# shibatch/rectdetect

Hardware: AMD Instinct MI355X
Metric: 1920x1080 frames/sec (higher is better)
Workload: dtype u8/i32/f32 (bit-exact integer + IEEE f32 stencil path)

## Files before the change

### rectdetect_amd/csrc/rd_k_front.hip

```cpp
#include <stdlib.h>
#include "rd_device.h"
#include "rd_kernels.h"
#include "rectdetect_hip.h"

#define RD_LUT_ATTR __device__
#include "rd_luts.h"

namespace {

using namespace rd;
using namespace rdpix;

struct P3 { float *p[3]; };
struct P3c { const float *p[3]; };
struct SrcZ { const uint8_t *p[RD_ZB_MAX]; };

inline int cdiv(int a, int b) { return (a + b - 1) / b; }
inline dim3 grid2(int iw, int ih) { return dim3(cdiv(iw, 64), cdiv(ih, 4)); }
const dim3 block2(64, 4);
inline int grid1(int n) { int g = cdiv(n, 256); return g < 1 ? 1 : g; }

__device__ __forceinline__ int lerp_lut(const unsigned short *t, int c) { return t[c >> 8] * (256 - (c & 255)) + t[(c >> 8) + 1] * (c & 255); }

__device__ __forceinline__ uint32_t plab_of(const unsigned short *s_s2l, const unsigned short *s_cf, const unsigned short *s_cf2, int b, int g, int r) {
  const int ib = s_s2l[b], ig = s_s2l[g], ir = s_s2l[r];
  const int cx = (((ir * 6758 + ig * 5859 + ib * 2956 + (1 << 14)) >> 15) * 34476 + (1 << 10)) >> 11;
  const int cy = ((ir * 3484 + ig * 11717 + ib * 1182) + (1 << 10)) >> 11;
  const int cz = (((ir * 317 + ig * 1953 + ib * 15569 + (1 << 14)) >> 15) * 30097 + (1 << 10)) >> 11;
  const int cl = ((lerp_lut(s_cf2, cy) >> 12) + 1) >> 1;
  const int fx = lerp_lut(s_cf, cx), fy = lerp_lut(s_cf, cy), fz = lerp_lut(s_cf, cz);
  const int fxy = (fx - fy + (1 << 7)) >> 8, fyz = (fy - fz + (1 << 7)) >> 8;
  const int ca = (fxy * 8031 + (134744072 + (1 << 17))) >> 18;
  const int cb = (fyz * 3213 + (134744072 + (1 << 17))) >> 18;
  uint32_t v = clampu((uint32_t)cb, 0u, 1023u);
  v = (v << 10) | clampu((uint32_t)ca, 0u, 1023u);
  v = (v << 12) | clampu((uint32_t)cl, 0u, 4095u);
  return v;
}

__global__ __launch_bounds__(256) void k_bgr2plab(uint32_t *__restrict__ out, const uint8_t *__restrict__ bgr, int iw, int ih, int ws) {
  __shared__ unsigned short s_s2l[RD_LUT_S2L_N], s_cf[RD_LUT_CF_N], s_cf2[RD_LUT_CF_N];
  const int tid = rd_ty() * 64 + threadIdx.x;
  for (int i = tid; i < RD_LUT_S2L_N; i += 256) s_s2l[i] = rd_lut_s2l[i];
  for (int i = tid; i < RD_LUT_CF_N; i += 256) { s_cf[i] = rd_lut_cfunc[i]; s_cf2[i] = rd_lut_cfunc2[i]; }
  __syncthreads();
  const int x = blockIdx.x * 64 + threadIdx.x;
  if (x >= iw) return;
  for (int r = 0; r < 4; r++) {
    const int y = (blockIdx.y * 4 + rd_ty()) * 4 + r;
    if (y >= ih) break;
    const uint8_t *p = bgr + (size_t)y * ws + x * 3;
    const int ib = s_s2l[p[0]], ig = s_s2l[p[1]], ir = s_s2l[p[2]];
    const int cx = (((ir * 6758 + ig * 5859 + ib * 2956 + (1 << 14)) >> 15) * 34476 + (1 << 10)) >> 11;
    const int cy = ((ir * 3484 + ig * 11717 + ib * 1182) + (1 << 10)) >> 11;
    const int cz = (((ir * 317 + ig * 1953 + ib * 15569 + (1 << 14)) >> 15) * 30097 + (1 << 10)) >> 11;
    const int cl = ((lerp_lut(s_cf2, cy) >> 12) + 1) >> 1;
    const int fx = lerp_lut(s_cf, cx), fy = lerp_lut(s_cf, cy), fz = lerp_lut(s_cf, cz);
    const int fxy = (fx - fy + (1 << 7)) >> 8, fyz = (fy - fz + (1 << 7)) >> 8;
    const int ca = (fxy * 8031 + (134744072 + (1 << 17))) >> 18;
    const int cb = (fyz * 3213 + (134744072 + (1 << 17))) >> 18;
    uint32_t v = clampu((uint32_t)cb, 0u, 1023u);
    v = (v << 10) | clampu((uint32_t)ca, 0u, 1023u);
    v = (v << 12) | clampu((uint32_t)cl, 0u, 4095u);
    out[y * iw + x] = v;
  }
}

__global__ __launch_bounds__(256) void k_bgr2plab_t(uint32_t *__restrict__ out, P3 dst, SrcZ srcz, int iw, int ih, int ws, size_t zs) {
  const uint8_t *__restrict__ bgr = srcz.p[blockIdx.z];
  RD_ZSHIFT(zs, out, dst.p[0], dst.p[1], dst.p[2]);
  __shared__ unsigned short s_s2l[RD_LUT_S2L_N], s_cf[RD_LUT_CF_N], s_cf2[RD_LUT_CF_N];
  __shared__ unsigned short tile[3][64][66];
  const int tid = rd_ty() * 64 + threadIdx.x;
  const int x0 = blockIdx.x * 64, y0 = blockIdx.y * 64;
  const int x = x0 + threadIdx.x;
  uint8_t pb[16], pg[16], pr[16];
#pragma unroll
  for (int k = 0; k < 16; k++) {
    const int y = y0 + rd_ty() + 4 * k;
    const uint8_t *p = bgr + ((x < iw && y < ih) ? (size_t)y * ws + x * 3 : 0);
    pb[k] = p[0]; pg[k] = p[1]; pr[k] = p[2];
  }
  for (int i = tid; i < RD_LUT_S2L_N; i += 256) s_s2l[i] = rd_lut_s2l[i];
  for (int i = tid; i < RD_LUT_CF_N; i += 256) { s_cf[i] = rd_lut_cfunc[i]; s_cf2[i] = rd_lut_cfunc2[i]; }
  __syncthreads();
#pragma unroll
  for (int k = 0; k < 16; k++) {
    const int r = rd_ty() + 4 * k;
    const int y = y0 + r;
    if (x >= iw || y >= ih) continue;
    const int ib = s_s2l[pb[k]], ig = s_s2l[pg[k]], ir = s_s2l[pr[k]];
    const int cx = (((ir * 6758 + ig * 5859 + ib * 2956 + (1 << 14)) >> 15) * 34476 + (1 << 10)) >> 11;
    const int cy = ((ir * 3484 + ig * 11717 + ib * 1182) + (1 << 10)) >> 11;
    const int cz = (((ir * 317 + ig * 1953 + ib * 15569 + (1 << 14)) >> 15) * 30097 + (1 << 10)) >> 11;
    const int cl = ((lerp_lut(s_cf2, cy) >> 12) + 1) >> 1;
    const int fx = lerp_lut(s_cf, cx), fy = lerp_lut(s_cf, cy), fz = lerp_lut(s_cf, cz);
    const int fxy = (fx - fy + (1 << 7)) >> 8, fyz = (fy - fz + (1 << 7)) >> 8;
    const int ca = (fxy * 8031 + (134744072 + (1 << 17))) >> 18;
    const int cb = (fyz * 3213 + (134744072 + (1 << 17))) >> 18;
    uint32_t v = clampu((uint32_t)cb, 0u, 1023u);
    v = (v << 10) | clampu((uint32_t)ca, 0u, 1023u);
    v = (v << 12) | clampu((uint32_t)cl, 0u, 4095u);
    out[y * iw + x] = v;
    tile[0][r][threadIdx.x] = (unsigned short)(v & 4095u); tile[1][r][threadIdx.x] = (unsigned short)((v >> 12) & 1023u); tile[2][r][threadIdx.x] = (unsigned short)((v >> 22) & 1023u);
  }
  __syncthreads();
  for (int r = rd_ty(); r < 64; r += 4) {
    const int ox = y0 + threadIdx.x, oy = x0 + r;
    if (ox < ih && oy < iw)
      for (int k = 0; k < 3; k++) ((unsigned short *)dst.p[k])[(size_t)oy * ih + ox] = tile[k][threadIdx.x][r];
  }
}

struct PixZ { const uint8_t *p[3][RD_ZB_MAX]; int pitch[3]; int wide; };

__device__ __forceinline__ uint32_t ld_bytes(const uint8_t *p, int n) {
  uint32_t w = 0;
#pragma unroll
  for (int i = 0; i < 4; i++) if (i < n) w |= (uint32_t)p[i] << (8 * i);
  return w;
}
template <int FMT> __device__ __forceinline__ void pix_load4(uint32_t (&w)[4], const uint8_t *p0, const uint8_t *p1, const uint8_t *p2, const int (&pitch)[3], int x, int y, int m, bool wide) {
  if (rdpix::bpp(FMT) == 3) {
    const uint8_t *q = p0 + (size_t)y * pitch[0] + 3 * x;
    if (wide && m == 4) { const uint32_t *q4 = (const uint32_t *)q; w[0] = q4[0]; w[1] = q4[1]; w[2] = q4[2]; }
    else for (int k = 0; k < 3; k++) w[k] = ld_bytes(q + 4 * k, 3 * m - 4 * k);
  } else if (rdpix::bpp(FMT) == 4) {
    const uint8_t *q = p0 + (size_t)y * pitch[0] + 4 * x;
    if (wide && m == 4) { const uint4 v = *(const uint4 *)q; w[0] = v.x; w[1] = v.y; w[2] = v.z; w[3] = v.w; }
    else for (int k = 0; k < 4; k++) w[k] = ld_bytes(q + 4 * k, k < m ? 4 : 0);
  } else {
    const uint8_t *q = p0 + (size_t)y * pitch[0] + x;
    const int c = (m + 1) >> 1;
    if (FMT == RD_PIX_NV12) {
      const uint8_t *uv = p1 + (size_t)(y >> 1) * pitch[1] + x;
      if (wide && m == 4) { w[0] = *(const uint32_t *)q; w[1] = *(const uint32_t *)uv; }
      else { w[0] = ld_bytes(q, m); w[1] = ld_bytes(uv, 2 * c); }
    } else {
      const uint8_t *u = p1 + (size_t)(y >> 1) * pitch[1] + (x >> 1), *v = p2 + (size_t)(y >> 1) * pitch[2] + (x >> 1);
      if (wide && m == 4) { w[0] = *(const uint32_t *)q; w[1] = (uint32_t)*(const unsigned short *)u | ((uint32_t)*(const unsigned short *)v << 16); }
      else { w[0] = ld_bytes(q, m); w[1] = ld_bytes(u, c) | (ld_bytes(v, c) << 16); }
    }
  }
}

template <int FMT> __device__ __forceinline__ void pix_bgr(const uint32_t (&w)[4], int j, int &b, int &g, int &r) {
  const auto byte = [&](int i) { return (int)((w[i >> 2] >> (8 * (i & 3))) & 255u); };
  if (!is_yuv(FMT)) {
    const int i = rdpix::bpp(FMT) * j, c[3] = { byte(i), byte(i + 1), byte(i + 2) };
    b = c[rb_swapped(FMT) ? 2 : 0]; g = c[1]; r = c[rb_swapped(FMT) ? 0 : 2];
  } else if (FMT == RD_PIX_NV12) yuv_bgr(byte(j), byte(4 + 2 * (j >> 1)), byte(5 + 2 * (j >> 1)), b, g, r);
  else yuv_bgr(byte(j), byte(4 + (j >> 1)), byte(6 + (j >> 1)), b, g, r);
}

template <int FMT>
__global__ __launch_bounds__(256) void k_pix2plab_t(uint32_t *__restrict__ out, P3 dst, PixZ src, int iw, int ih, size_t zs) {
  const int z = blockIdx.z;
  const uint8_t *__restrict__ p0 = src.p[0][z], *__restrict__ p1 = src.p[1][z], *__restrict__ p2 = src.p[2][z];
  RD_ZSHIFT(zs, out, dst.p[0], dst.p[1], dst.p[2]);
  __shared__ unsigned short s_s2l[RD_LUT_S2L_N], s_cf[RD_LUT_CF_N], s_cf2[RD_LUT_CF_N];
  __shared__ unsigned short tile[3][64][66];
  const int tid = rd_ty() * 64 + threadIdx.x;
  const int x0 = blockIdx.x * 64, y0 = blockIdx.y * 64;
  const int cx = (tid & 15) * 4, r0 = tid >> 4;
  const int x = x0 + cx, m = min(iw - x, 4);
  uint32_t w[4][4] = {};
#pragma unroll
  for (int k = 0; k < 4; k++) {
    const int y = y0 + r0 + 16 * k;
    if (m > 0 && y < ih) pix_load4<FMT>(w[k], p0, p1, p2, src.pitch, x, y, m, src.wide != 0);
  }
  for (int i = tid; i < RD_LUT_S2L_N; i += 256) s_s2l[i] = rd_lut_s2l[i];
  for (int i = tid; i < RD_LUT_CF_N; i += 256) { s_cf[i] = rd_lut_cfunc[i]; s_cf2[i] = rd_lut_cfunc2[i]; }
  __syncthreads();
#pragma unroll
  for (int k = 0; k < 4; k++) {
    const int r = r0 + 16 * k, y = y0 + r;
    if (m <= 0 || y >= ih) continue;
    uint32_t v[4];
#pragma unroll
    for (int j = 0; j < 4; j++) {
      int b, g, rr;
      pix_bgr<FMT>(w[k], j, b, g, rr);
      v[j] = plab_of(s_s2l, s_cf, s_cf2, b, g, rr);
      tile[0][r][cx + j] = (unsigned short)(v[j] & 4095u); tile[1][r][cx + j] = (unsigned short)((v[j] >> 12) & 1023u); tile[2][r][cx + j] = (unsigned short)((v[j] >> 22) & 1023u);
    }
    uint32_t *o = out + (size_t)y * iw + x;
    if (m == 4 && (iw & 3) == 0) *(uint4 *)o = make_uint4(v[0], v[1], v[2], v[3]);
    else for (int j = 0; j < m; j++) o[j] = v[j];
  }
  __syncthreads();
  for (int r = rd_ty(); r < 64; r += 4) {
    const int ox = y0 + threadIdx.x, oy = x0 + r;
    if (ox < ih && oy < iw)
      for (int k = 0; k < 3; k++) ((unsigned short *)dst.p[k])[(size_t)oy * ih + ox] = tile[k][threadIdx.x][r];
  }
}

template <int FMT> struct HalfW { static constexpr int row = 2 * rdpix::bpp(FMT), n = is_yuv(FMT) ? 6 : 2 * row; };

template <int FMT> __device__ __forceinline__ void pix_load_half(uint32_t (&w)[HalfW<FMT>::n], const uint8_t *p0, const uint8_t *p1, const uint8_t *p2, const int (&pitch)[3], int x, int y, int m, bool wide) {
  constexpr int RW = HalfW<FMT>::row;
  const bool full = wide && m == 4;
  if (!is_yuv(FMT)) {
    constexpr int bpp = rdpix::bpp(FMT);
    const uint8_t *q = p0 + (size_t)(2 * y) * pitch[0] + (size_t)(2 * x) * bpp;
#pragma unroll
    for (int r = 0; r < 2; r++, q += pitch[0]) {
      if (full) {
        if (bpp == 4) { const uint4 a = ((const uint4 *)q)[0], b = ((const uint4 *)q)[1]; w[RW * r] = a.x; w[RW * r + 1] = a.y; w[RW * r + 2] = a.z; w[RW * r + 3] = a.w; w[RW * r + 4] = b.x; w[RW * r + 5] = b.y; w[RW * r + 6] = b.z; w[RW * r + 7] = b.w; }
        else { const uint2 a = ((const uint2 *)q)[0], b = ((const uint2 *)q)[1], c = ((const uint2 *)q)[2]; w[RW * r] = a.x; w[RW * r + 1] = a.y; w[RW * r + 2] = b.x; w[RW * r + 3] = b.y; w[RW * r + 4] = c.x; w[RW * r + 5] = c.y; }
      } else {
#pragma unroll
        for (int k = 0; k < RW; k++) w[RW * r + k] = ld_bytes(q + 4 * k, 2 * m * bpp - 4 * k);
      }
    }
  } else {
    const uint8_t *q = p0 + (size_t)(2 * y) * pitch[0] + 2 * x;
#pragma unroll
    for (int r = 0; r < 2; r++, q += pitch[0]) {
      if (full) { const uint2 a = *(const uint2 *)q; w[2 * r] = a.x; w[2 * r + 1] = a.y; }
      else { w[2 * r] = ld_bytes(q, 2 * m); w[2 * r + 1] = ld_bytes(q + 4, 2 * m - 4); }
    }
    if (FMT == RD_PIX_NV12) {
      const uint8_t *uv = p1 + (size_t)y * pitch[1] + 2 * x;
      if (full) { const uint2 a = *(const uint2 *)uv; w[4] = a.x; w[5] = a.y; }
      else { w[4] = ld_bytes(uv, 2 * m); w[5] = ld_bytes(uv + 4, 2 * m - 4); }
    } else {
      const uint8_t *u = p1 + (size_t)y * pitch[1] + x, *v = p2 + (size_t)y * pitch[2] + x;
      if (full) { w[4] = *(const uint32_t *)u; w[5] = *(const uint32_t *)v; }
      else { w[4] = ld_bytes(u, m); w[5] = ld_bytes(v, m); }
    }
  }
}

template <int FMT> __device__ __forceinline__ void pix_bgr_half(const uint32_t (&w)[HalfW<FMT>::n], int j, int &b, int &g, int &r) {
  constexpr int RW = HalfW<FMT>::row;
  const auto byte = [&](int i) { return (int)((w[i >> 2] >> (8 * (i & 3))) & 255u); };
  b = g = r = 2;
#pragma unroll
  for (int t = 0; t < 4; t++) {
    const int sx = 2 * j + (t & 1), sr = t >> 1;
    int pb, pg, pr;
    if (!is_yuv(FMT)) {
      const int i = 4 * RW * sr + rdpix::bpp(FMT) * sx, c[3] = { byte(i), byte(i + 1), byte(i + 2) };
      pb = c[rb_swapped(FMT) ? 2 : 0]; pg = c[1]; pr = c[rb_swapped(FMT) ? 0 : 2];
    } else if (FMT == RD_PIX_NV12) yuv_bgr(byte(8 * sr + sx), byte(16 + 2 * j), byte(17 + 2 * j), pb, pg, pr);
    else yuv_bgr(byte(8 * sr + sx), byte(16 + j), byte(20 + j), pb, pg, pr);
    b += pb; g += pg; r += pr;
  }
  b >>= 2; g >>= 2; r >>= 2;
}

template <int FMT>
__global__ __launch_bounds__(256) void k_pix2plab_half_t(uint32_t *__restrict__ out, P3 dst, PixZ src, int iw, int ih, size_t zs) {
  const int z = blockIdx.z;
  const uint8_t *__restrict__ p0 = src.p[0][z], *__restrict__ p1 = src.p[1][z], *__restrict__ p2 = src.p[2][z];
  RD_ZSHIFT(zs, out, dst.p[0], dst.p[1], dst.p[2]);
  __shared__ unsigned short s_s2l[RD_LUT_S2L_N], s_cf[RD_LUT_CF_N], s_cf2[RD_LUT_CF_N];
  __shared__ unsigned short tile[3][64][66];
  const int tid = rd_ty() * 64 + threadIdx.x;
  const int x0 = blockIdx.x * 64, y0 = blockIdx.y * 64;
  const int cx = (tid & 15) * 4, r0 = tid >> 4;
  const int x = x0 + cx, m = min(iw - x, 4);
  uint32_t w[4][HalfW<FMT>::n] = {};
#pragma unroll
  for (int k = 0; k < 4; k++) {
    const int y = y0 + r0 + 16 * k;
    if (m > 0 && y < ih) pix_load_half<FMT>(w[k], p0, p1, p2, src.pitch, x, y, m, src.wide != 0);
  }
  for (int i = tid; i < RD_LUT_S2L_N; i += 256) s_s2l[i] = rd_lut_s2l[i];
  for (int i = tid; i < RD_LUT_CF_N; i += 256) { s_cf[i] = rd_lut_cfunc[i]; s_cf2[i] = rd_lut_cfunc2[i]; }
  __syncthreads();
#pragma unroll
  for (int k = 0; k < 4; k++) {
    const int r = r0 + 16 * k, y = y0 + r;
    if (m <= 0 || y >= ih) continue;
    uint32_t v[4];
#pragma unroll
    for (int j = 0; j < 4; j++) {
      int b, g, rr;
      pix_bgr_half<FMT>(w[k], j, b, g, rr);
      v[j] = plab_of(s_s2l, s_cf, s_cf2, b, g, rr);
      tile[0][r][cx + j] = (unsigned short)(v[j] & 4095u); tile[1][r][cx + j] = (unsigned short)((v[j] >> 12) & 1023u); tile[2][r][cx + j] = (unsigned short)((v[j] >> 22) & 1023u);
    }
    uint32_t *o = out + (size_t)y * iw + x;
    if (m == 4 && (iw & 3) == 0) *(uint4 *)o = make_uint4(v[0], v[1], v[2], v[3]);
    else for (int j = 0; j < m; j++) o[j] = v[j];
  }
  __syncthreads();
  for (int r = rd_ty(); r < 64; r += 4) {
    const int ox = y0 + threadIdx.x, oy = x0 + r;
    if (ox < ih && oy < iw)
      for (int k = 0; k < 3; k++) ((unsigned short *)dst.p[k])[(size_t)oy * ih + ox] = tile[k][threadIdx.x][r];
  }
}

template <typename LD, typename ST> __device__ __forceinline__ void ew4(int n, LD ld, ST st) {
  const int stride = gridDim.x * blockDim.x;
  int i = blockIdx.x * blockDim.x + threadIdx.x;
  for (; i + 3 * stride < n; i += 4 * stride) {
    const auto v0 = ld(i), v1 = ld(i + stride), v2 = ld(i + 2 * stride), v3 = ld(i + 3 * stride);
    st(i, v0); st(i + stride, v1); st(i + 2 * stride, v2); st(i + 3 * stride, v3);
  }
  for (; i < n; i += stride) st(i, ld(i));
}

__global__ void k_unpack_plab(float *__restrict__ L, float *__restrict__ a, float *__restrict__ b, const uint32_t *__restrict__ in, int n) {
  for (int i = blockIdx.x * blockDim.x + threadIdx.x; i < n; i += gridDim.x * blockDim.x) {
    float l, aa, bb;
    unpack_lab(in[i], l, aa, bb);
    L[i] = l; a[i] = aa; b[i] = bb;
  }
}

__global__ void k_pack_plab(uint32_t *__restrict__ out, const float *__restrict__ L, const float *__restrict__ a, const float *__restrict__ b, int n) {
  ew4(n, [=](int i) { return make_float3(L[i], a[i], b[i]); }, [=](int i, float3 v) { out[i] = pack_lab(v.x, v.y, v.z); });
}

template <int MODE>
__global__ __launch_bounds__(256) void k_transpose(P3 dst, P3c src, P3c fwd, P3c bwd, const uint32_t *__restrict__ plab, int np, int W, int H, const int *only_if) {
  if (only_if && *only_if == 0) return;
  __shared__ float tile[3][64][65];
  const int x0 = blockIdx.x * 64, y0 = blockIdx.y * 64;
  for (int r = rd_ty(); r < 64; r += 4) {
    const int x = x0 + threadIdx.x, y = y0 + r;
    if (x < W && y < H) {
      const size_t i = (size_t)y * W + x;
// ... 141 lines not shown
          if (xin && yy >= s0 && yy < s0 + 7) IIR_OUT(tl + (size_t)(3 * 7 + yy - s0) * W) = d;
          IIR_SHIFT(cur[j]);
        }
#pragma unroll
        for (int j = 0; j < IIR_CH; j++) cur[j] = nxt[j];
      }
    }
  }
  if (TOUT) {
    __syncthreads();
    const int rows = s1 - s0;
    for (int col = anti; col < 64; col += 2) {
      const int xx = blockIdx.x * 64 + col;
      if (xx >= W) break;
      float *__restrict__ o = dk + (size_t)xx * H + s0;
      for (int r = lane; r < rows; r += 64) at32(o, (unsigned)r) = fwt[r * IF_PITCH + col];
    }
  }
}

__device__ __forceinline__ unsigned iir_off(unsigned o) { asm("" : "+v"(o)); return o; }
template <typename T> __device__ __forceinline__ __attribute__((address_space(1))) T *iir_uni(T *p) {
  __attribute__((address_space(1))) T *g = (__attribute__((address_space(1))) T *)p;
  asm("" : "+s"(g));
  return g;
}
#ifndef IIR_PCH
#define IIR_PCH 16
#endif
#ifndef IF_TB
#define IF_TB 32
#endif
#define IF_TP (64 + 64 / IF_TB)
#ifdef IF_WPE
#define IF_WPE_ATTR __attribute__((amdgpu_waves_per_eu(IF_WPE)))
#else
#define IF_WPE_ATTR
#endif
template <int TOUT, int IF_ROWS, int SRC16>
__global__ __launch_bounds__(128) IF_WPE_ATTR void k_iir_fused(P3 dst, P3c src, float *__restrict__ tails, int W, int H, int nchunks, int *bad, int np, size_t zs) {
  constexpr int HALF = IF_ROWS / 2, CH = IIR_PCH, CPI = 64 / IF_TB;
  static_assert(CH >= 8 && IF_WU % CH == 0 && HALF % CH == 0 && HALF % IF_TB == 0 && 64 % IF_TB == 0, "whole chunks and whole batches, half a block per phase");
  __shared__ float swp[2 * 14 * 64];
  __shared__ float stg[TOUT ? 2 * IF_TB * IF_TP : 1];
  const int lane = threadIdx.x & 63, anti = __builtin_amdgcn_readfirstlane((int)(threadIdx.x >> 6));
  const int fz = __builtin_amdgcn_readfirstlane((int)(blockIdx.y / np)), k = blockIdx.y - fz * np, c = blockIdx.z;
  float *dk = k == 0 ? dst.p[0] : (k == 1 ? dst.p[1] : dst.p[2]);
  const float *sk = k == 0 ? src.p[0] : (k == 1 ? src.p[1] : src.p[2]);
  { const size_t rd_zoff_ = (size_t)fz * zs; RD_ZS1(dk); RD_ZS1(sk); RD_ZS1(tails); RD_ZS1(bad); }
  if (blockIdx.x == 0 && k == 0 && blockIdx.z == 0 && threadIdx.x == 0) *bad = 0;
  const int x = blockIdx.x * 64 + lane;
  const bool xin = x < W;
  typedef typename iir_src<SRC16>::T TS;
  const TS *__restrict__ in = (const TS *)sk;
  const unsigned xs = (unsigned)(xin ? x : W - 1) * (unsigned)sizeof(TS), x4 = (unsigned)(xin ? x : W - 1) * 4u;
#undef IIR_ROW
#undef IIR_OUT
#define IIR_ROW(ptr) (*(const TS *)((const char *)(ptr) + xo_))
#define IIR_OUT(ptr) (*(float *)((char *)(ptr) + iir_off(x4)))
  const float sc = k == 0 ? 1.0f / 4096 : 1.0f / 1024, hf = k == 0 ? 0.5f / 4096 : 0.5f / 1024;
  const int s0 = c * IF_ROWS, s1 = s0 + IF_ROWS, mid = s0 + HALF;
  float *__restrict__ tl = tails + ((size_t)(k * nchunks + c) * 4 * 7) * W;
  const long rs = anti ? -(long)W : (long)W;
  float cur[CH], nxt[CH], park[HALF];
#define IIR_PSTEPS(...)                                                                                                  \
      _Pragma("unroll") for (int j = 0; j < CH; j++) {                                                                   \
        IIR_STEP(cur[j]);                                                                                                \
        __VA_ARGS__;                                                                                                     \
        IIR_SHIFT(cur[j]);                                                                                               \
      }                                                                                                                  \
      _Pragma("unroll") for (int j = 0; j < CH; j++) cur[j] = nxt[j];
#define IIR_PCHUNK(MORE, NEXT, NSTEP, ...)                                                                               \
    {                                                                                                                    \
      if (MORE) { const TS *n_ = (NEXT); const unsigned xo_ = iir_off(xs); _Pragma("unroll") for (int j = 0; j < CH; j++) { nxt[j] = IIR_LD(IIR_ROW(iir_uni(n_))); n_ += (NSTEP); } } \
      IIR_PSTEPS(__VA_ARGS__)                                                                                            \
    }
#define IIR_PARK(dst, v) asm("v_mov_b32 %0, %1" : "=v"(dst) : "v"(v))
  IIR_STATE;
  const TS *p = in + (size_t)(anti ? s1 - 1 : s0) * W;
  const TS *const pb = in + (size_t)(anti ? mid : mid - 1) * W;
  float *const tw = tl + (size_t)(anti ? 2 * 7 + 6 : 0) * W;
#define IIR_WTAIL if (j >= CH - 7 && xin) IIR_OUT(iir_uni(tw + (long)(j - (CH - 7)) * rs)) = d
  if (anti ? s1 + IF_WU <= H : s0 - IF_WU >= 0) {
    const TS *w = p - IF_WU * rs;
    { const unsigned xo_ = iir_off(xs);
#pragma unroll
      for (int j = 0; j < CH; j++) cur[j] = IIR_LD(IIR_ROW(iir_uni(w + (long)j * rs))); }
    for (int q = 0; q < IF_WU / CH - 1; q++) { IIR_PCHUNK(1, w + CH * rs, rs, (void)0); w += CH * rs; }
    IIR_PCHUNK(1, p, rs, IIR_WTAIL);
  } else {
    const int dy = anti ? -1 : 1, y0 = anti ? s1 - 1 + IF_WU : s0 - IF_WU;
    const unsigned xo_ = iir_off(xs);
    auto eld = [&](int yy) -> float {
      const int yc = clampi(yy, -IIR_WARM, H + IIR_WARM);
      const float v = IIR_LD(IIR_ROW(iir_uni(in + (size_t)mirror1(yc, H) * W)));
      return yy == yc ? v : 0.0f;
    };
#define IIR_PCHUNK_E(YN, ...) { _Pragma("unroll") for (int j = 0; j < CH; j++) nxt[j] = eld((YN) + j * dy); IIR_PSTEPS(__VA_ARGS__) }
#pragma unroll
    for (int j = 0; j < CH; j++) cur[j] = eld(y0 + j * dy);
    for (int q = 0; q < IF_WU / CH - 1; q++) IIR_PCHUNK_E(y0 + (q + 1) * CH * dy, (void)0)
    IIR_PCHUNK(1, p, rs, IIR_WTAIL);
  }
#undef IIR_WTAIL
#pragma unroll
  for (int q = 0; q < HALF / CH; q++) {
    const bool last = q == HALF / CH - 1;
    IIR_PCHUNK(1, last ? pb : p + CH * rs, last ? -rs : rs, IIR_PARK(park[q * CH + j], d)); p += CH * rs;
  }
  {
    float *mine = swp + anti * (14 * 64) + lane, *theirs = swp + (anti ^ 1) * (14 * 64) + lane;
#define IIR_SWAP(n, q) mine[(2 * n) * 64] = q.x; mine[(2 * n + 1) * 64] = q.y;
    IIR_SWAP(0, q1) IIR_SWAP(1, q2) IIR_SWAP(2, q3) IIR_SWAP(3, q4) IIR_SWAP(4, q5) IIR_SWAP(5, q6) IIR_SWAP(6, q7)
#undef IIR_SWAP
    __syncthreads();
#define IIR_SWAP(n, q) q.x = theirs[(2 * n) * 64]; q.y = theirs[(2 * n + 1) * 64];
    IIR_SWAP(0, q1) IIR_SWAP(1, q2) IIR_SWAP(2, q3) IIR_SWAP(3, q4) IIR_SWAP(4, q5) IIR_SWAP(5, q6) IIR_SWAP(6, q7)
#undef IIR_SWAP
  }
  p = pb;
  float *const tt = tl + (size_t)(anti ? 1 * 7 : 3 * 7 + 6) * W;
  float *o = dk + (size_t)(anti ? mid : mid - 1) * W;
  float *const st = stg + (TOUT ? anti * (IF_TB * IF_TP) : 0);
  const int br = lane % IF_TB, bc = lane / IF_TB;
  const float *const sl = st + (anti ? br : IF_TB - 1 - br) * IF_TP + bc;
  const unsigned bo = ((unsigned)bc * (unsigned)H + (unsigned)br) * 4u;
#pragma unroll
  for (int q = 0; q < HALF / CH; q++) {
    const bool last = q == HALF / CH - 1;
    IIR_PCHUNK(!last, p - CH * rs, -rs, {
      const int i = q * CH + j;
      const float r = (park[HALF - 1 - i] + d) - cur[j] * IIR_C0;
      if (TOUT) st[(i % IF_TB) * IF_TP + lane] = r; else if (xin) IIR_OUT(iir_uni(o - (long)j * rs)) = r;
      if (i >= HALF - 7 && xin) IIR_OUT(iir_uni(tt - (long)(i - (HALF - 7)) * rs)) = d;
      if (TOUT && i % IF_TB == IF_TB - 1) {
        __builtin_amdgcn_fence(__ATOMIC_RELEASE, "wavefront"); __builtin_amdgcn_wave_barrier(); __builtin_amdgcn_fence(__ATOMIC_ACQUIRE, "wavefront");
        const int lowest = anti ? mid + (i / IF_TB) * IF_TB : mid - (i / IF_TB + 1) * IF_TB;
        float *const ob = dk + (size_t)(blockIdx.x * 64) * H + lowest;
        _Pragma("unroll") for (int n = 0; n < IF_TB; n++)
          if ((int)blockIdx.x * 64 + n * CPI + bc < W) *(float *)((char *)iir_uni(ob + (size_t)(n * CPI) * H) + bo) = sl[n * CPI];
        __builtin_amdgcn_fence(__ATOMIC_RELEASE, "wavefront"); __builtin_amdgcn_wave_barrier(); __builtin_amdgcn_fence(__ATOMIC_ACQUIRE, "wavefront");
      }
    });
    p -= CH * rs; if (!TOUT) o -= CH * rs;
  }
#undef IIR_PCHUNK
#undef IIR_PCHUNK_E
#undef IIR_PSTEPS
#undef IIR_PARK
}

#undef IIR_LD
#undef IIR_ROW
#undef IIR_OUT

#define IC_CH 4
template <int TOUT, int SRC16, int EAGER>
__global__ __launch_bounds__(64 * IC_CH) void k_iir_check_fix(P3 dst, P3c src, P3 fwd, const float *__restrict__ tails, int *bad, int W, int H, int nchunks, int IF_ROWS, int force, int np, size_t zs) {
  const int x = blockIdx.x * 64 + threadIdx.x;
  const int k = blockIdx.y % np, c = blockIdx.z * IC_CH + rd_ty();
  if (c >= nchunks) return;
  float *dk = k == 0 ? dst.p[0] : (k == 1 ? dst.p[1] : dst.p[2]), *fk = k == 0 ? fwd.p[0] : (k == 1 ? fwd.p[1] : fwd.p[2]);
  const float *sk = k == 0 ? src.p[0] : (k == 1 ? src.p[1] : src.p[2]);
  { const size_t rd_zoff_ = (size_t)(blockIdx.y / np) * zs; RD_ZS1(dk); RD_ZS1(sk); RD_ZS1(fk); RD_ZS1(tails); RD_ZS1(bad); }
  if (x >= W) return;
  const int s0 = c * IF_ROWS, s1 = (c == nchunks - 1) ? H : s0 + IF_ROWS;
  const float *me = tails + ((size_t)(k * nchunks + c) * 4 * 7) * W + x;
  bool differ = force != 0 && c == 0;
  const bool chk_f = c > 0 && s0 - IF_WU > -IIR_WARM;
  const bool chk_b = c < nchunks - 1 && s1 - 1 + IF_WU < H + IIR_WARM;
  const float *pv = tails + ((size_t)(k * nchunks + (chk_f ? c - 1 : c)) * 4 * 7) * W + x;
  const float *nx = tails + ((size_t)(k * nchunks + (chk_b ? c + 1 : c)) * 4 * 7) * W + x;
  if (EAGER) {
    unsigned a[14], b[14];
#pragma unroll
    for (int j = 0; j < 7; j++) {
      a[j] = __float_as_uint(me[(size_t)(0 * 7 + j) * W]); b[j] = __float_as_uint(pv[(size_t)(1 * 7 + j) * W]);
      a[7 + j] = __float_as_uint(me[(size_t)(2 * 7 + j) * W]); b[7 + j] = __float_as_uint(nx[(size_t)(3 * 7 + j) * W]);
    }
    unsigned df = 0, db = 0;
#pragma unroll
    for (int j = 0; j < 7; j++) { df |= a[j] ^ b[j]; db |= a[7 + j] ^ b[7 + j]; }
    differ = differ || (chk_f && df != 0) || (chk_b && db != 0);
  } else {
    if (chk_f) {
#pragma unroll
      for (int j = 0; j < 7; j++) differ = differ || (__float_as_uint(me[(size_t)(0 * 7 + j) * W]) != __float_as_uint(pv[(size_t)(1 * 7 + j) * W]));
    }
    if (chk_b) {
#pragma unroll
      for (int j = 0; j < 7; j++) differ = differ || (__float_as_uint(me[(size_t)(2 * 7 + j) * W]) != __float_as_uint(nx[(size_t)(3 * 7 + j) * W]));
    }
  }
  if (!differ) return;
  atomicOr(bad, 1);
  typedef typename iir_src<SRC16>::T TS;
  const TS *__restrict__ in = (const TS *)sk + x;
  const float sc = k == 0 ? 1.0f / 4096 : 1.0f / 1024, hf = k == 0 ? 0.5f / 4096 : 0.5f / 1024;
  float *fw = fk + x;
  {
    IIR_STATE;
    for (int yy = -IIR_WARM; yy < H; yy++) {
      const float i0 = iir_field<SRC16>(in[(size_t)mirror1(yy, H) * W], sc, hf);
// ... 380 lines not shown
  }
  return z;
}
void pix2plab_transposed(hipStream_t s, int fmt, uint32_t *out, float *const dst[3], const uint8_t *const (*planes)[3], const int pitch[3], int iw, int ih, int nz, size_t zs) {
  const P3 d = { { dst[0], dst[1], dst[2] } };
  const PixZ z = pixz_of(planes, pitch, nz);
  const dim3 grid(cdiv(iw, 64), cdiv(ih, 64), nz);
  const bool known = fmt != RD_PIX_BGR && dispatch(fmt, [&](auto f) {
    if constexpr (f.value != RD_PIX_BGR) hipLaunchKernelGGL(k_pix2plab_t<f.value>, grid, block2, 0, s, out, d, z, iw, ih, zs);
  });
  if (!known) abort();
}
void pix2plab_half_transposed(hipStream_t s, int fmt, uint32_t *out, float *const dst[3], const uint8_t *const (*planes)[3], const int pitch[3], int iw, int ih, int nz, size_t zs) {
  const P3 d = { { dst[0], dst[1], dst[2] } };
  const PixZ z = pixz_of(planes, pitch, nz);
  const dim3 grid(cdiv(iw, 64), cdiv(ih, 64), nz);
  if (!dispatch(fmt, [&](auto f) { hipLaunchKernelGGL(k_pix2plab_half_t<f.value>, grid, block2, 0, s, out, d, z, iw, ih, zs); })) abort();
}
void unpack_plab(hipStream_t s, float *L, float *a, float *b, const uint32_t *in, int n) {
  hipLaunchKernelGGL(k_unpack_plab, dim3(ew_grid(n)), dim3(256), 0, s, L, a, b, in, n);
}
void pack_plab(hipStream_t s, uint32_t *out, const float *L, const float *a, const float *b, int n) {
  hipLaunchKernelGGL(k_pack_plab, dim3(ew_grid(n)), dim3(256), 0, s, out, L, a, b, n);
}

static P3 mk3(float *const p[3], int np) { P3 r = { { nullptr, nullptr, nullptr } }; for (int k = 0; k < np; k++) r.p[k] = p[k]; return r; }
static P3c mk3c(const float *const p[3], int np) { P3c r = { { nullptr, nullptr, nullptr } }; for (int k = 0; k < np; k++) r.p[k] = p[k]; return r; }

void transpose_f(hipStream_t s, float *const dst[3], const float *const src[3], int np, int W, int H) {
  P3c z = { { nullptr, nullptr, nullptr } };
  hipLaunchKernelGGL(k_transpose<0>, dim3(cdiv(W, 64), cdiv(H, 64)), block2, 0, s, mk3(dst, np), mk3c(src, np), z, z, (const uint32_t *)nullptr, np, W, H, (const int *)nullptr);
}
static int if_pick_rows(int np, int W, int H, int transpose_out, int nz) {
  (void)np; (void)W; (void)H;
  (void)transpose_out;
#ifndef IF_GROUP_ROWS
#define IF_GROUP_ROWS 128
#endif
  if (nz > 1) return IF_GROUP_ROWS;
  return 64;
}

size_t iir_pass_scratch_floats(int np, int W, int H) { return (size_t)np * if_nchunks(H, IF_ROWS_MIN) * 4 * 7 * W; }

void iir_blur_pass(hipStream_t s, float *const dst[3], const float *const src[3], float *const fwd[3], float *const bwd[3], int np, int W, int H,
                   int transpose_out, float *tails, int *bad, int src16, int nz, size_t zs) {
  const int rows = if_pick_rows(np, W, H, transpose_out, nz);
  const int nchunks = if_nchunks(H, rows);
  const int nf = (H - (nchunks - 1) * rows == rows) ? nchunks : nchunks - 1;
  const dim3 grid(cdiv(W, 64), np * nz, nchunks);
  const dim3 fgrid(grid.x, grid.y, nf), egrid(grid.x, grid.y, nchunks - nf);
#define IF_LAUNCH(T, R, S16) { if (nf > 0) hipLaunchKernelGGL((k_iir_fused<T, R, S16>), fgrid, dim3(128), 0, s, mk3(dst, np), mk3c(src, np), tails, W, H, nchunks, bad, np, zs); \
    if (nf < nchunks) hipLaunchKernelGGL((k_iir_fused_edge<T, R, S16>), egrid, dim3(128), 0, s, mk3(dst, np), mk3c(src, np), tails, W, H, nchunks, nf, bad, np, zs); }
#define IF_LAUNCH_R(R) { if (transpose_out && src16) IF_LAUNCH(1, R, 1) else if (transpose_out) IF_LAUNCH(1, R, 0) else IF_LAUNCH(0, R, 0) }
  switch (rows) {
    case 64: IF_LAUNCH_R(64); break;
#if IF_GROUP_ROWS != 64 && IF_GROUP_ROWS != 128
    case IF_GROUP_ROWS: IF_LAUNCH_R(IF_GROUP_ROWS); break;
#endif
    default: IF_LAUNCH_R(128); break;
  }
#undef IF_LAUNCH_R
#undef IF_LAUNCH
  if (nchunks > 1) {
    const dim3 cgrid(grid.x, grid.y, cdiv(nchunks, IC_CH)), cblock(64, IC_CH);
    const int force = getenv("RD_IIR_FORCE_FIX") ? 1 : 0;
#define IC_LAUNCH(T, S16, E) hipLaunchKernelGGL((k_iir_check_fix<T, S16, E>), cgrid, cblock, 0, s, mk3(dst, np), mk3c(src, np), mk3(fwd, np), (const float *)tails, bad, W, H, nchunks, rows, force, np, zs)
    if (nz > 1) { if (transpose_out && src16) IC_LAUNCH(1, 1, 0); else if (transpose_out) IC_LAUNCH(1, 0, 0); else IC_LAUNCH(0, 0, 0); }
    else { if (transpose_out && src16) IC_LAUNCH(1, 1, 1); else if (transpose_out) IC_LAUNCH(1, 0, 1); else IC_LAUNCH(0, 0, 1); }
#undef IC_LAUNCH
  }
  (void)bwd;
}

void iir_blur_lines(hipStream_t s, float *dst, const float *src, float *fw, float *bw, int W, int H, int r) {
  hipLaunchKernelGGL(k_iir_line, dim3(cdiv(W, 64)), dim3(64, 2), 0, s, dst, src, fw, bw, W, H, r);
}

void convert_bgr_lumaf(hipStream_t s, uint8_t *out, const float *in, float f, int iw, int ih, int ws) {
  hipLaunchKernelGGL(k_convert_bgr_lumaf, grid2(iw, ih), block2, 0, s, out, in, f, iw, ih, ws);
}
void convert_bgr_labeli(hipStream_t s, uint8_t *out, const int *in, int bgc, int iw, int ih, int ws) {
  hipLaunchKernelGGL(k_convert_bgr_labeli, grid2(iw, ih), block2, 0, s, out, in, bgc, iw, ih, ws);
}
void plab2bgr(hipStream_t s, uint8_t *out, const uint32_t *in, int iw, int ih, int ws) {
  hipLaunchKernelGGL(k_plab2bgr, grid2(iw, ih), block2, 0, s, out, in, iw, ih, ws);
}
void edge_f(hipStream_t s, float *out, const float *in, int iw, int ih) {
  hipLaunchKernelGGL(k_edge_f, grid2(iw, ih), block2, 0, s, out, in, iw, ih);
}
void edgevec_plab(hipStream_t s, float *vxy, const uint32_t *in, int iw, int ih) {
  hipLaunchKernelGGL(k_edgevec_plab, grid2(iw, ih), block2, 0, s, (float2 *)vxy, in, iw, ih);
}
void thincubic(hipStream_t s, float *out, const float *in, const float *vxy, int iw, int ih) {
  hipLaunchKernelGGL(k_thincubic, grid2(iw, ih), block2, 0, s, out, in, (const float2 *)vxy, iw, ih);
}
void edgevec(hipStream_t s, float *vxy, const float *in, int iw, int ih, uint32_t *pack_out, const float *a, const float *b, int nz, size_t zs) {
  hipLaunchKernelGGL(k_edgevec, dim3(cdiv(iw, 64), cdiv(ih, 4 * EV_PX), nz), block2, 0, s, (float2 *)vxy, in, iw, ih, pack_out, a, b, zs);
}
void edge_plab(hipStream_t s, float *out, const uint32_t *in, int iw, int ih, int nz, size_t zs) {
// ... 29 lines not shown
```

Measured before the change: 3434.

## Pack Lab LUT pairs, single-word transpose tile, and 120-row IIR chunks for 1080-high frames

The Lab conversion tables are restaged as packed pairs of adjacent cfunc/cfunc2 entries in one uint2, so each interpolation needs one shared load instead of two, and the three 16-bit transpose tiles are merged into one 32-bit tile unpacked at write-out. The batched (nz>1) non-transposed IIR pass now uses 120-row chunks with a 12-row chunk size and 36-row run-in when H divides by 120 but not 128, as with 1080. That removes the ragged edge-chunk launch and lets the check/fix kernel receive the run-in length as a parameter. The trade-off is more chunks, each with relatively more warm-up work, plus an extra template instantiation.

```diff
diff --git a/rectdetect_amd/csrc/rd_k_front.hip b/rectdetect_amd/csrc/rd_k_front.hip
--- a/rectdetect_amd/csrc/rd_k_front.hip
+++ b/rectdetect_amd/csrc/rd_k_front.hip
@@ -20,15 +20,44 @@
 const dim3 block2(64, 4);
 inline int grid1(int n) { int g = cdiv(n, 256); return g < 1 ? 1 : g; }
 
-__device__ __forceinline__ int lerp_lut(const unsigned short *t, int c) { return t[c >> 8] * (256 - (c & 255)) + t[(c >> 8) + 1] * (c & 255); }
-
-__device__ __forceinline__ uint32_t plab_of(const unsigned short *s_s2l, const unsigned short *s_cf, const unsigned short *s_cf2, int b, int g, int r) {
-  const int ib = s_s2l[b], ig = s_s2l[g], ir = s_s2l[r];
-  const int cx = (((ir * 6758 + ig * 5859 + ib * 2956 + (1 << 14)) >> 15) * 34476 + (1 << 10)) >> 11;
-  const int cy = ((ir * 3484 + ig * 11717 + ib * 1182) + (1 << 10)) >> 11;
-  const int cz = (((ir * 317 + ig * 1953 + ib * 15569 + (1 << 14)) >> 15) * 30097 + (1 << 10)) >> 11;
-  const int cl = ((lerp_lut(s_cf2, cy) >> 12) + 1) >> 1;
-  const int fx = lerp_lut(s_cf, cx), fy = lerp_lut(s_cf, cy), fz = lerp_lut(s_cf, cz);
+#define RD_CF_IMAX 1024
+#define RD_CFP_N (RD_LUT_CF_N - 1)
+#define RD_S2L_WHITE 32768
+constexpr int lab_cx(int ir, int ig, int ib) { return (((ir * 6758 + ig * 5859 + ib * 2956 + (1 << 14)) >> 15) * 34476 + (1 << 10)) >> 11; }
+constexpr int lab_cy(int ir, int ig, int ib) { return ((ir * 3484 + ig * 11717 + ib * 1182) + (1 << 10)) >> 11; }
+constexpr int lab_cz(int ir, int ig, int ib) { return (((ir * 317 + ig * 1953 + ib * 15569 + (1 << 14)) >> 15) * 30097 + (1 << 10)) >> 11; }
+static_assert((lab_cx(RD_S2L_WHITE, RD_S2L_WHITE, RD_S2L_WHITE) >> 8) == RD_CF_IMAX && (lab_cz(RD_S2L_WHITE, RD_S2L_WHITE, RD_S2L_WHITE) >> 8) == RD_CF_IMAX &&
+              (lab_cy(RD_S2L_WHITE, RD_S2L_WHITE, RD_S2L_WHITE) >> 8) == RD_CF_IMAX - 1 && RD_CF_IMAX < RD_CFP_N && RD_CF_IMAX + 1 < RD_LUT_CF_N,
+              "the largest index white reaches has its pair entry");
+struct LabTables { uint2 cfp[RD_CFP_N]; unsigned short s2l[RD_LUT_S2L_N]; };
+
+__device__ __forceinline__ void lab_tables_stage(LabTables &t, int tid) {
+  constexpr int NP = (RD_CFP_N + 255) / 256, NS = (RD_LUT_S2L_N + 255) / 256;
+  unsigned short a[NP][4], l[NS];
+#pragma unroll
+  for (int k = 0; k < NP; k++) {
+    const int i = min(tid + 256 * k, RD_CFP_N - 1);
+    a[k][0] = rd_lut_cfunc[i]; a[k][1] = rd_lut_cfunc[i + 1]; a[k][2] = rd_lut_cfunc2[i]; a[k][3] = rd_lut_cfunc2[i + 1];
+  }
+#pragma unroll
+  for (int k = 0; k < NS; k++) l[k] = rd_lut_s2l[min(tid + 256 * k, RD_LUT_S2L_N - 1)];
+#pragma unroll
+  for (int k = 0; k < NP; k++)
+    if (tid + 256 * k < RD_CFP_N) t.cfp[tid + 256 * k] = make_uint2((uint32_t)a[k][0] | ((uint32_t)a[k][1] << 16), (uint32_t)a[k][2] | ((uint32_t)a[k][3] << 16));
+#pragma unroll
+  for (int k = 0; k < NS; k++)
+    if (tid + 256 * k < RD_LUT_S2L_N) t.s2l[tid + 256 * k] = l[k];
+}
+
+__device__ __forceinline__ int lerp_pair(uint32_t e, int c) { return (int)(e & 0xffffu) * (256 - (c & 255)) + (int)(e >> 16) * (c & 255); }
+
+__device__ __forceinline__ uint32_t plab_of(const LabTables &t, int b, int g, int r) {
+  const int ib = t.s2l[b], ig = t.s2l[g], ir = t.s2l[r];
+  const int cx = lab_cx(ir, ig, ib), cy = lab_cy(ir, ig, ib), cz = lab_cz(ir, ig, ib);
+  const uint2 ey = t.cfp[cy >> 8];
+  const uint32_t ex = t.cfp[cx >> 8].x, ez = t.cfp[cz >> 8].x;
+  const int cl = ((lerp_pair(ey.y, cy) >> 12) + 1) >> 1;
+  const int fx = lerp_pair(ex, cx), fy = lerp_pair(ey.x, cy), fz = lerp_pair(ez, cz);
   const int fxy = (fx - fy + (1 << 7)) >> 8, fyz = (fy - fz + (1 << 7)) >> 8;
   const int ca = (fxy * 8031 + (134744072 + (1 << 17))) >> 18;
   const int cb = (fyz * 3213 + (134744072 + (1 << 17))) >> 18;
@@ -38,11 +67,22 @@
   return v;
 }
 
+#define LAB_TILE_P 65
+__device__ __forceinline__ void lab_tile_out(const uint32_t (&tile)[64][LAB_TILE_P], const P3 &dst, int x0, int y0, int iw, int ih) {
+  for (int r = rd_ty(); r < 64; r += 4) {
+    const int ox = y0 + threadIdx.x, oy = x0 + r;
+    if (ox < ih && oy < iw) {
+      const uint32_t v = tile[threadIdx.x][r];
+      const size_t o = (size_t)oy * ih + ox;
+      ((unsigned short *)dst.p[0])[o] = (unsigned short)(v & 4095u); ((unsigned short *)dst.p[1])[o] = (unsigned short)((v >> 12) & 1023u); ((unsigned short *)dst.p[2])[o] = (unsigned short)((v >> 22) & 1023u);
+    }
+  }
+}
+
 __global__ __launch_bounds__(256) void k_bgr2plab(uint32_t *__restrict__ out, const uint8_t *__restrict__ bgr, int iw, int ih, int ws) {
-  __shared__ unsigned short s_s2l[RD_LUT_S2L_N], s_cf[RD_LUT_CF_N], s_cf2[RD_LUT_CF_N];
+  __shared__ LabTables tb;
   const int tid = rd_ty() * 64 + threadIdx.x;
-  for (int i = tid; i < RD_LUT_S2L_N; i += 256) s_s2l[i] = rd_lut_s2l[i];
-  for (int i = tid; i < RD_LUT_CF_N; i += 256) { s_cf[i] = rd_lut_cfunc[i]; s_cf2[i] = rd_lut_cfunc2[i]; }
+  lab_tables_stage(tb, tid);
   __syncthreads();
   const int x = blockIdx.x * 64 + threadIdx.x;
   if (x >= iw) return;
@@ -50,27 +90,15 @@
     const int y = (blockIdx.y * 4 + rd_ty()) * 4 + r;
     if (y >= ih) break;
     const uint8_t *p = bgr + (size_t)y * ws + x * 3;
-    const int ib = s_s2l[p[0]], ig = s_s2l[p[1]], ir = s_s2l[p[2]];
-    const int cx = (((ir * 6758 + ig * 5859 + ib * 2956 + (1 << 14)) >> 15) * 34476 + (1 << 10)) >> 11;
-    const int cy = ((ir * 3484 + ig * 11717 + ib * 1182) + (1 << 10)) >> 11;
-    const int cz = (((ir * 317 + ig * 1953 + ib * 15569 + (1 << 14)) >> 15) * 30097 + (1 << 10)) >> 11;
-    const int cl = ((lerp_lut(s_cf2, cy) >> 12) + 1) >> 1;
-    const int fx = lerp_lut(s_cf, cx), fy = lerp_lut(s_cf, cy), fz = lerp_lut(s_cf, cz);
-    const int fxy = (fx - fy + (1 << 7)) >> 8, fyz = (fy - fz + (1 << 7)) >> 8;
-    const int ca = (fxy * 8031 + (134744072 + (1 << 17))) >> 18;
-    const int cb = (fyz * 3213 + (134744072 + (1 << 17))) >> 18;
-    uint32_t v = clampu((uint32_t)cb, 0u, 1023u);
-    v = (v << 10) | clampu((uint32_t)ca, 0u, 1023u);
-    v = (v << 12) | clampu((uint32_t)cl, 0u, 4095u);
-    out[y * iw + x] = v;
+    out[y * iw + x] = plab_of(tb, p[0], p[1], p[2]);
   }
 }
 
 __global__ __launch_bounds__(256) void k_bgr2plab_t(uint32_t *__restrict__ out, P3 dst, SrcZ srcz, int iw, int ih, int ws, size_t zs) {
   const uint8_t *__restrict__ bgr = srcz.p[blockIdx.z];
   RD_ZSHIFT(zs, out, dst.p[0], dst.p[1], dst.p[2]);
-  __shared__ unsigned short s_s2l[RD_LUT_S2L_N], s_cf[RD_LUT_CF_N], s_cf2[RD_LUT_CF_N];
-  __shared__ unsigned short tile[3][64][66];
+  __shared__ LabTables tb;
+  __shared__ uint32_t tile[64][LAB_TILE_P];
   const int tid = rd_ty() * 64 + threadIdx.x;
   const int x0 = blockIdx.x * 64, y0 = blockIdx.y * 64;
   const int x = x0 + threadIdx.x;
@@ -81,35 +109,19 @@
     const uint8_t *p = bgr + ((x < iw && y < ih) ? (size_t)y * ws + x * 3 : 0);
     pb[k] = p[0]; pg[k] = p[1]; pr[k] = p[2];
   }
-  for (int i = tid; i < RD_LUT_S2L_N; i += 256) s_s2l[i] = rd_lut_s2l[i];
-  for (int i = tid; i < RD_LUT_CF_N; i += 256) { s_cf[i] = rd_lut_cfunc[i]; s_cf2[i] = rd_lut_cfunc2[i]; }
+  lab_tables_stage(tb, tid);
   __syncthreads();
 #pragma unroll
   for (int k = 0; k < 16; k++) {
     const int r = rd_ty() + 4 * k;
     const int y = y0 + r;
     if (x >= iw || y >= ih) continue;
-    const int ib = s_s2l[pb[k]], ig = s_s2l[pg[k]], ir = s_s2l[pr[k]];
-    const int cx = (((ir * 6758 + ig * 5859 + ib * 2956 + (1 << 14)) >> 15) * 34476 + (1 << 10)) >> 11;
-    const int cy = ((ir * 3484 + ig * 11717 + ib * 1182) + (1 << 10)) >> 11;
-    const int cz = (((ir * 317 + ig * 1953 + ib * 15569 + (1 << 14)) >> 15) * 30097 + (1 << 10)) >> 11;
-    const int cl = ((lerp_lut(s_cf2, cy) >> 12) + 1) >> 1;
-    const int fx = lerp_lut(s_cf, cx), fy = lerp_lut(s_cf, cy), fz = lerp_lut(s_cf, cz);
-    const int fxy = (fx - fy + (1 << 7)) >> 8, fyz = (fy - fz + (1 << 7)) >> 8;
-    const int ca = (fxy * 8031 + (134744072 + (1 << 17))) >> 18;
-    const int cb = (fyz * 3213 + (134744072 + (1 << 17))) >> 18;
-    uint32_t v = clampu((uint32_t)cb, 0u, 1023u);
-    v = (v << 10) | clampu((uint32_t)ca, 0u, 1023u);
-    v = (v << 12) | clampu((uint32_t)cl, 0u, 4095u);
+    const uint32_t v = plab_of(tb, pb[k], pg[k], pr[k]);
     out[y * iw + x] = v;
-    tile[0][r][threadIdx.x] = (unsigned short)(v & 4095u); tile[1][r][threadIdx.x] = (unsigned short)((v >> 12) & 1023u); tile[2][r][threadIdx.x] = (unsigned short)((v >> 22) & 1023u);
+    tile[r][threadIdx.x] = v;
   }
   __syncthreads();
-  for (int r = rd_ty(); r < 64; r += 4) {
-    const int ox = y0 + threadIdx.x, oy = x0 + r;
-    if (ox < ih && oy < iw)
-      for (int k = 0; k < 3; k++) ((unsigned short *)dst.p[k])[(size_t)oy * ih + ox] = tile[k][threadIdx.x][r];
-  }
+  lab_tile_out(tile, dst, x0, y0, iw, ih);
 }
 
 struct PixZ { const uint8_t *p[3][RD_ZB_MAX]; int pitch[3]; int wide; };
@@ -158,8 +170,8 @@
   const int z = blockIdx.z;
   const uint8_t *__restrict__ p0 = src.p[0][z], *__restrict__ p1 = src.p[1][z], *__restrict__ p2 = src.p[2][z];
   RD_ZSHIFT(zs, out, dst.p[0], dst.p[1], dst.p[2]);
-  __shared__ unsigned short s_s2l[RD_LUT_S2L_N], s_cf[RD_LUT_CF_N], s_cf2[RD_LUT_CF_N];
-  __shared__ unsigned short tile[3][64][66];
+  __shared__ LabTables tb;
+  __shared__ uint32_t tile[64][LAB_TILE_P];
   const int tid = rd_ty() * 64 + threadIdx.x;
   const int x0 = blockIdx.x * 64, y0 = blockIdx.y * 64;
   const int cx = (tid & 15) * 4, r0 = tid >> 4;
@@ -170,8 +182,7 @@
     const int y = y0 + r0 + 16 * k;
     if (m > 0 && y < ih) pix_load4<FMT>(w[k], p0, p1, p2, src.pitch, x, y, m, src.wide != 0);
   }
-  for (int i = tid; i < RD_LUT_S2L_N; i += 256) s_s2l[i] = rd_lut_s2l[i];
-  for (int i = tid; i < RD_LUT_CF_N; i += 256) { s_cf[i] = rd_lut_cfunc[i]; s_cf2[i] = rd_lut_cfunc2[i]; }
+  lab_tables_stage(tb, tid);
   __syncthreads();
 #pragma unroll
   for (int k = 0; k < 4; k++) {
@@ -182,19 +193,15 @@
     for (int j = 0; j < 4; j++) {
       int b, g, rr;
       pix_bgr<FMT>(w[k], j, b, g, rr);
-      v[j] = plab_of(s_s2l, s_cf, s_cf2, b, g, rr);
-      tile[0][r][cx + j] = (unsigned short)(v[j] & 4095u); tile[1][r][cx + j] = (unsigned short)((v[j] >> 12) & 1023u); tile[2][r][cx + j] = (unsigned short)((v[j] >> 22) & 1023u);
+      v[j] = plab_of(tb, b, g, rr);
+      tile[r][cx + j] = v[j];
     }
     uint32_t *o = out + (size_t)y * iw + x;
     if (m == 4 && (iw & 3) == 0) *(uint4 *)o = make_uint4(v[0], v[1], v[2], v[3]);
     else for (int j = 0; j < m; j++) o[j] = v[j];
   }
   __syncthreads();
-  for (int r = rd_ty(); r < 64; r += 4) {
-    const int ox = y0 + threadIdx.x, oy = x0 + r;
-    if (ox < ih && oy < iw)
-      for (int k = 0; k < 3; k++) ((unsigned short *)dst.p[k])[(size_t)oy * ih + ox] = tile[k][threadIdx.x][r];
-  }
+  lab_tile_out(tile, dst, x0, y0, iw, ih);
 }
 
 template <int FMT> struct HalfW { static constexpr int row = 2 * rdpix::bpp(FMT), n = is_yuv(FMT) ? 6 : 2 * row; };
@@ -257,8 +264,8 @@
   const int z = blockIdx.z;
   const uint8_t *__restrict__ p0 = src.p[0][z], *__restrict__ p1 = src.p[1][z], *__restrict__ p2 = src.p[2][z];
   RD_ZSHIFT(zs, out, dst.p[0], dst.p[1], dst.p[2]);
-  __shared__ unsigned short s_s2l[RD_LUT_S2L_N], s_cf[RD_LUT_CF_N], s_cf2[RD_LUT_CF_N];
-  __shared__ unsigned short tile[3][64][66];
+  __shared__ LabTables tb;
+  __shared__ uint32_t tile[64][LAB_TILE_P];
   const int tid = rd_ty() * 64 + threadIdx.x;
   const int x0 = blockIdx.x * 64, y0 = blockIdx.y * 64;
   const int cx = (tid & 15) * 4, r0 = tid >> 4;
@@ -269,8 +276,7 @@
     const int y = y0 + r0 + 16 * k;
     if (m > 0 && y < ih) pix_load_half<FMT>(w[k], p0, p1, p2, src.pitch, x, y, m, src.wide != 0);
   }
-  for (int i = tid; i < RD_LUT_S2L_N; i += 256) s_s2l[i] = rd_lut_s2l[i];
-  for (int i = tid; i < RD_LUT_CF_N; i += 256) { s_cf[i] = rd_lut_cfunc[i]; s_cf2[i] = rd_lut_cfunc2[i]; }
+  lab_tables_stage(tb, tid);
   __syncthreads();
 #pragma unroll
   for (int k = 0; k < 4; k++) {
@@ -281,19 +287,15 @@
     for (int j = 0; j < 4; j++) {
       int b, g, rr;
       pix_bgr_half<FMT>(w[k], j, b, g, rr);
-      v[j] = plab_of(s_s2l, s_cf, s_cf2, b, g, rr);
-      tile[0][r][cx + j] = (unsigned short)(v[j] & 4095u); tile[1][r][cx + j] = (unsigned short)((v[j] >> 12) & 1023u); tile[2][r][cx + j] = (unsigned short)((v[j] >> 22) & 1023u);
+      v[j] = plab_of(tb, b, g, rr);
+      tile[r][cx + j] = v[j];
     }
     uint32_t *o = out + (size_t)y * iw + x;
     if (m == 4 && (iw & 3) == 0) *(uint4 *)o = make_uint4(v[0], v[1], v[2], v[3]);
     else for (int j = 0; j < m; j++) o[j] = v[j];
   }
   __syncthreads();
-  for (int r = rd_ty(); r < 64; r += 4) {
-    const int ox = y0 + threadIdx.x, oy = x0 + r;
-    if (ox < ih && oy < iw)
-      for (int k = 0; k < 3; k++) ((unsigned short *)dst.p[k])[(size_t)oy * ih + ox] = tile[k][threadIdx.x][r];
-  }
+  lab_tile_out(tile, dst, x0, y0, iw, ih);
 }
 
 template <typename LD, typename ST> __device__ __forceinline__ void ew4(int n, LD ld, ST st) {
@@ -501,15 +503,21 @@
 #define IF_TB 32
 #endif
 #define IF_TP (64 + 64 / IF_TB)
+#define IF_ROWS_120 120
+#define IF_CH_120 12
+#ifndef IF_WU_120
+#define IF_WU_120 36
+#endif
 #ifdef IF_WPE
 #define IF_WPE_ATTR __attribute__((amdgpu_waves_per_eu(IF_WPE)))
 #else
 #define IF_WPE_ATTR
 #endif
-template <int TOUT, int IF_ROWS, int SRC16>
+template <int TOUT, int IF_ROWS, int SRC16, int CH = IIR_PCH, int WU = IF_WU>
 __global__ __launch_bounds__(128) IF_WPE_ATTR void k_iir_fused(P3 dst, P3c src, float *__restrict__ tails, int W, int H, int nchunks, int *bad, int np, size_t zs) {
-  constexpr int HALF = IF_ROWS / 2, CH = IIR_PCH, CPI = 64 / IF_TB;
-  static_assert(CH >= 8 && IF_WU % CH == 0 && HALF % CH == 0 && HALF % IF_TB == 0 && 64 % IF_TB == 0, "whole chunks and whole batches, half a block per phase");
+  constexpr int HALF = IF_ROWS / 2, CPI = 64 / IF_TB;
+  static_assert(CH >= 8 && WU % CH == 0 && WU >= IIR_WARM && HALF % CH == 0 && 64 % IF_TB == 0, "whole chunks per half and whole chunks of run-in, half a block per phase");
+  static_assert(!TOUT || HALF % IF_TB == 0, "transposed output leaves in whole batches");
   __shared__ float swp[2 * 14 * 64];
   __shared__ float stg[TOUT ? 2 * IF_TB * IF_TP : 1];
   const int lane = threadIdx.x & 63, anti = __builtin_amdgcn_readfirstlane((int)(threadIdx.x >> 6));
@@ -550,15 +558,15 @@
   const TS *const pb = in + (size_t)(anti ? mid : mid - 1) * W;
   float *const tw = tl + (size_t)(anti ? 2 * 7 + 6 : 0) * W;
 #define IIR_WTAIL if (j >= CH - 7 && xin) IIR_OUT(iir_uni(tw + (long)(j - (CH - 7)) * rs)) = d
-  if (anti ? s1 + IF_WU <= H : s0 - IF_WU >= 0) {
-    const TS *w = p - IF_WU * rs;
+  if (anti ? s1 + WU <= H : s0 - WU >= 0) {
+    const TS *w = p - WU * rs;
     { const unsigned xo_ = iir_off(xs);
 #pragma unroll
       for (int j = 0; j < CH; j++) cur[j] = IIR_LD(IIR_ROW(iir_uni(w + (long)j * rs))); }
-    for (int q = 0; q < IF_WU / CH - 1; q++) { IIR_PCHUNK(1, w + CH * rs, rs, (void)0); w += CH * rs; }
+    for (int q = 0; q < WU / CH - 1; q++) { IIR_PCHUNK(1, w + CH * rs, rs, (void)0); w += CH * rs; }
     IIR_PCHUNK(1, p, rs, IIR_WTAIL);
   } else {
-    const int dy = anti ? -1 : 1, y0 = anti ? s1 - 1 + IF_WU : s0 - IF_WU;
+    const int dy = anti ? -1 : 1, y0 = anti ? s1 - 1 + WU : s0 - WU;
     const unsigned xo_ = iir_off(xs);
     auto eld = [&](int yy) -> float {
       const int yc = clampi(yy, -IIR_WARM, H + IIR_WARM);
@@ -568,7 +576,7 @@
 #define IIR_PCHUNK_E(YN, ...) { _Pragma("unroll") for (int j = 0; j < CH; j++) nxt[j] = eld((YN) + j * dy); IIR_PSTEPS(__VA_ARGS__) }
 #pragma unroll
     for (int j = 0; j < CH; j++) cur[j] = eld(y0 + j * dy);
-    for (int q = 0; q < IF_WU / CH - 1; q++) IIR_PCHUNK_E(y0 + (q + 1) * CH * dy, (void)0)
+    for (int q = 0; q < WU / CH - 1; q++) IIR_PCHUNK_E(y0 + (q + 1) * CH * dy, (void)0)
     IIR_PCHUNK(1, p, rs, IIR_WTAIL);
   }
 #undef IIR_WTAIL
@@ -625,7 +633,7 @@
 
 #define IC_CH 4
 template <int TOUT, int SRC16, int EAGER>
-__global__ __launch_bounds__(64 * IC_CH) void k_iir_check_fix(P3 dst, P3c src, P3 fwd, const float *__restrict__ tails, int *bad, int W, int H, int nchunks, int IF_ROWS, int force, int np, size_t zs) {
+__global__ __launch_bounds__(64 * IC_CH) void k_iir_check_fix(P3 dst, P3c src, P3 fwd, const float *__restrict__ tails, int *bad, int W, int H, int nchunks, int IF_ROWS, int wu, int force, int np, size_t zs) {
   const int x = blockIdx.x * 64 + threadIdx.x;
   const int k = blockIdx.y % np, c = blockIdx.z * IC_CH + rd_ty();
   if (c >= nchunks) return;
@@ -636,8 +644,8 @@
   const int s0 = c * IF_ROWS, s1 = (c == nchunks - 1) ? H : s0 + IF_ROWS;
   const float *me = tails + ((size_t)(k * nchunks + c) * 4 * 7) * W + x;
   bool differ = force != 0 && c == 0;
-  const bool chk_f = c > 0 && s0 - IF_WU > -IIR_WARM;
-  const bool chk_b = c < nchunks - 1 && s1 - 1 + IF_WU < H + IIR_WARM;
+  const bool chk_f = c > 0 && s0 - wu > -IIR_WARM;
+  const bool chk_b = c < nchunks - 1 && s1 - 1 + wu < H + IIR_WARM;
   const float *pv = tails + ((size_t)(k * nchunks + (chk_f ? c - 1 : c)) * 4 * 7) * W + x;
   const float *nx = tails + ((size_t)(k * nchunks + (chk_b ? c + 1 : c)) * 4 * 7) * W + x;
   if (EAGER) {
@@ -1084,12 +1092,11 @@
   hipLaunchKernelGGL(k_transpose<0>, dim3(cdiv(W, 64), cdiv(H, 64)), block2, 0, s, mk3(dst, np), mk3c(src, np), z, z, (const uint32_t *)nullptr, np, W, H, (const int *)nullptr);
 }
 static int if_pick_rows(int np, int W, int H, int transpose_out, int nz) {
-  (void)np; (void)W; (void)H;
-  (void)transpose_out;
+  (void)np; (void)W;
 #ifndef IF_GROUP_ROWS
 #define IF_GROUP_ROWS 128
 #endif
-  if (nz > 1) return IF_GROUP_ROWS;
+  if (nz > 1) return (H % IF_GROUP_ROWS != 0 && H % IF_ROWS_120 == 0 && !transpose_out) ? IF_ROWS_120 : IF_GROUP_ROWS;
   return 64;
 }
 
@@ -1110,14 +1117,18 @@
 #if IF_GROUP_ROWS != 64 && IF_GROUP_ROWS != 128
     case IF_GROUP_ROWS: IF_LAUNCH_R(IF_GROUP_ROWS); break;
 #endif
+    case IF_ROWS_120:
+      hipLaunchKernelGGL((k_iir_fused<0, IF_ROWS_120, 0, IF_CH_120, IF_WU_120>), fgrid, dim3(128), 0, s, mk3(dst, np), mk3c(src, np), tails, W, H, nchunks, bad, np, zs);
+      break;
     default: IF_LAUNCH_R(128); break;
   }
+  const int wu = rows == IF_ROWS_120 ? IF_WU_120 : IF_WU;
 #undef IF_LAUNCH_R
 #undef IF_LAUNCH
   if (nchunks > 1) {
     const dim3 cgrid(grid.x, grid.y, cdiv(nchunks, IC_CH)), cblock(64, IC_CH);
     const int force = getenv("RD_IIR_FORCE_FIX") ? 1 : 0;
-#define IC_LAUNCH(T, S16, E) hipLaunchKernelGGL((k_iir_check_fix<T, S16, E>), cgrid, cblock, 0, s, mk3(dst, np), mk3c(src, np), mk3(fwd, np), (const float *)tails, bad, W, H, nchunks, rows, force, np, zs)
+#define IC_LAUNCH(T, S16, E) hipLaunchKernelGGL((k_iir_check_fix<T, S16, E>), cgrid, cblock, 0, s, mk3(dst, np), mk3c(src, np), mk3(fwd, np), (const float *)tails, bad, W, H, nchunks, rows, wu, force, np, zs)
     if (nz > 1) { if (transpose_out && src16) IC_LAUNCH(1, 1, 0); else if (transpose_out) IC_LAUNCH(1, 0, 0); else IC_LAUNCH(0, 0, 0); }
     else { if (transpose_out && src16) IC_LAUNCH(1, 1, 1); else if (transpose_out) IC_LAUNCH(1, 0, 1); else IC_LAUNCH(0, 0, 1); }
 #undef IC_LAUNCH
```

After: 3447 (median of 6 runs). No clear change (+0.4%).
